# od-liu/CS3602-LLM-Inference-Acceleration

Hardware: NVIDIA B200
Metric: kv_compress_step_throughput (higher is better)
Workload: dtype bf16

## Files before the change

### cs3602-llm-inference-acceleration_b200/csrc/kvc_device.cuh

```cuda
#pragma once
#include <cuda_bf16.h>
#include <cuda_fp16.h>
#include <cuda_runtime.h>
#include <stdint.h>

#include <type_traits>

#include "kvc.h"

namespace kvc {

constexpr int kHistBits = 11;
constexpr int kHistBins = 1 << kHistBits;
constexpr int kMiscInts = 128;
constexpr int kMaxPoolHalo = 32;

constexpr int kMiscBin = 0;
constexpr int kMiscBelow = 1;
constexpr int kMiscMaxRaw = 2;
constexpr int kMiscWarpA = 32;
constexpr int kMiscWarpB = 64;
constexpr int kMiscHalo = 96;

struct CarryDev {
    char* acc;
    int64_t asb, ash;
    int32_t group, prev;
};
static_assert(sizeof(CarryDev) == 32, "CarryDev is part of the kernel parameters");

struct LayerDev {
    const char* k_in;
    const char* v_in;
    char* k_out;
    char* v_out;
    int32_t* idx_out;
    const int32_t* idx_in;
    int64_t ksb, ksh, kss;
    int64_t vsb, vsh, vss;
    int32_t S, sink, lo, hi, ksel, tail, score, pool;
    const char* n_in;
    int64_t nsb, nsh;
    CarryDev carry;
};
static_assert(sizeof(LayerDev) == 184, "LayerDev is passed by value in kernel params");

struct BatchDev {
    int32_t B, H;
    int32_t idx_cap;
    int32_t cpr;
    int32_t pad0, pad1;
    int32_t nsw;
    int32_t off_hist, off_idx, off_keys, off_stage;
    int32_t upc;
    char* ws;
    int64_t ws_unit;
    int64_t ws_keys;
    LayerDev layers[KVC_MAX_LAYERS_PER_LAUNCH];
};
static_assert(sizeof(BatchDev) < 32 * 1024, "kernel parameters are limited to 32 KB");

template <int DT>
struct Traits;
template <>
struct Traits<KVC_DTYPE_F32> {
    using Key = uint32_t;
    static constexpr int kElemBytes = 4;
    static constexpr int kKeyBits = 32;
    __device__ static __forceinline__ uint32_t to_raw(float x) { return __float_as_uint(x); }
    __device__ static __forceinline__ float from_raw(uint32_t r) { return __uint_as_float(r); }
    __device__ static __forceinline__ float sumsq(int4 v, float acc) {
        float a = __int_as_float(v.x), b = __int_as_float(v.y), c = __int_as_float(v.z), d = __int_as_float(v.w);
        acc = fmaf(a, a, acc);
        acc = fmaf(b, b, acc);
        acc = fmaf(c, c, acc);
        acc = fmaf(d, d, acc);
        return acc;
    }
};
template <>
struct Traits<KVC_DTYPE_BF16> {
    using Key = uint16_t;
    static constexpr int kElemBytes = 2;
    static constexpr int kKeyBits = 16;
    __device__ static __forceinline__ uint32_t to_raw(float x) {
        return (uint32_t)__bfloat16_as_ushort(__float2bfloat16_rn(x));
    }
    __device__ static __forceinline__ float from_raw(uint32_t r) { return __uint_as_float(r << 16); }
    __device__ static __forceinline__ float sumsq(int4 v, float acc) {
        const uint32_t w[4] = {(uint32_t)v.x, (uint32_t)v.y, (uint32_t)v.z, (uint32_t)v.w};
#pragma unroll
        for (int i = 0; i < 4; ++i) {
            float lo = __uint_as_float(w[i] << 16);
            float hi = __uint_as_float(w[i] & 0xffff0000u);
            acc = fmaf(lo, lo, acc);
            acc = fmaf(hi, hi, acc);
        }
        return acc;
    }
};
template <>
struct Traits<KVC_DTYPE_F16> {
    using Key = uint16_t;
    static constexpr int kElemBytes = 2;
    static constexpr int kKeyBits = 16;
    __device__ static __forceinline__ uint32_t to_raw(float x) {
        return (uint32_t)__half_as_ushort(__float2half_rn(x));
    }
    __device__ static __forceinline__ float from_raw(uint32_t r) {
        return __half2float(__ushort_as_half((unsigned short)r));
// ... 416 lines not shown
```

### cs3602-llm-inference-acceleration_b200/csrc/kvc_fused_tma.cuh

```cuda
#pragma once
#include "kvc_device.cuh"
#include "kvc_tma.cuh"

namespace kvc {

__host__ __device__ constexpr int swz_bits(int cpr) { return (cpr % 8 == 0) ? 3 : (cpr % 4 == 0) ? 2 : (cpr % 2 == 0) ? 1 : 0; }

template <int DT, int CPR>
__device__ __forceinline__ float row_sumsq_smem(uint32_t row_addr, int lane, int cpr) {
    using Tr = Traits<DT>;
    if constexpr (CPR == 0) {
        float tot = 0.f;
        for (int c = 0; c < cpr; ++c) {
            const float a = Tr::sumsq(lds128(row_addr + c * 16), 0.f);
            tot = (c == 0) ? a : tot + a;
        }
        return tot;
    } else {
        constexpr int SB = swz_bits(CPR);
        constexpr int G = 1 << SB;
        const int x = (lane >> (3 - SB)) & (G - 1);
        uint32_t base[G];
#pragma unroll
        for (int m = 0; m < G; ++m) base[m] = row_addr + (uint32_t)(((m ^ x) - m) * 16);
        float acc[CPR];
#pragma unroll
        for (int c = 0; c < CPR; ++c) acc[c] = Tr::sumsq(lds128(base[c & (G - 1)] + c * 16), 0.f);
        float tot = 0.f;
#pragma unroll
        for (int g = 0; g < CPR / G; ++g) {
#pragma unroll
            for (int s = 1; s < G; s <<= 1) {
#pragma unroll
                for (int m = 0; m < G; m += 2 * s) acc[g * G + m] += acc[g * G + m + s];
            }
            tot = (g == 0) ? acc[0] : tot + acc[g * G];
        }
        return tot;
    }
}

__device__ __forceinline__ void warp_load_rows(uint32_t slot, uint32_t bar, const char* src, int rows, bool dense,
                                               int lane, int rb) {
    const bool in = lane < rows;
    const unsigned long long a = (unsigned long long)src;
    const unsigned long long prev = __shfl_up_sync(0xffffffffu, a, 1);
    const bool head = in && (lane == 0 || !dense || a != prev + (unsigned)rb);
    const uint32_t heads = __ballot_sync(0xffffffffu, head);
    if (lane == 0) mbar_arrive_expect_tx(bar, (uint32_t)(rows * rb));
    __syncwarp();
    if (head) {
        const uint32_t later = heads & ~((2u << lane) - 1u);
        const int next = later ? (__ffs(later) - 1) : rows;
        bulk_g2s(slot + (uint32_t)(lane * rb), src, (uint32_t)((next - lane) * rb), bar);
    }
}

struct KeepMap {
    const int32_t* sidx;
    int sink, ksel, tail0;
    __device__ __forceinline__ int operator()(int j) const {
        return j < sink ? j : (j < sink + ksel ? sidx[j - sink] : j + tail0);
    }
};

template <typename Key, int NT>
__device__ __forceinline__ void carry_unit(const CarryDev& c, const KeepMap& src_row, int C, int b, int h) {
    char* base = c.acc + (int64_t)b * c.asb + (int64_t)h * c.group * c.ash;
    const int n = c.group * C;
    for (int e0 = 0; e0 < n; e0 += NT) {
        const int e = e0 + (int)threadIdx.x;
        Key* row = nullptr;
        int i = 0;
        Key val = 0;
        bool write = false;
        if (e < n) {
            const int g = e / C;
            i = e - g * C;
            const int s = src_row(i);
            row = reinterpret_cast<Key*>(base + (int64_t)g * c.ash);
            write = s != i || s >= c.prev;
            if (write && s < c.prev) val = row[s];
        }
        __syncthreads();
        if (write) row[i] = val;
    }
}

__device__ __forceinline__ void gather_unit(const KeepMap& src_row, int C, const char* kbase, const char* vbase,
                                            int64_t kss, int64_t vss, char* ko, char* vo, int rb, uint32_t slot,
                                            uint32_t bar, uint32_t& parity, int stage, int nstage, int lane) {
    const bool kdense = kss == rb, vdense = vss == rb;
    const int nbc = (C + 31) >> 5;
    for (int t = stage; t < 2 * nbc; t += nstage) {
        const bool isv = t >= nbc;
        const int j0 = (isv ? t - nbc : t) << 5;
        const int rows = min(32, C - j0);
        const int row = lane < rows ? src_row(j0 + lane) : 0;
        const char* src = isv ? vbase + (int64_t)row * vss : kbase + (int64_t)row * kss;
        warp_load_rows(slot, bar, src, rows, isv ? vdense : kdense, lane, rb);
        mbar_wait(bar, parity);
        parity ^= 1;
        if (lane == 0) {
            bulk_s2g((isv ? vo : ko) + (int64_t)j0 * rb, slot, (uint32_t)(rows * rb));
            bulk_commit();
            bulk_wait_read<0>();
        }
        __syncwarp();
    }
}

template <int DT, int NT>
__device__ __forceinline__ void keys_from_values(const typename Traits<DT>::Key* src, int R, int score,
                                                 typename Traits<DT>::Key* keys, uint32_t* hist, int32_t* misc) {
    using Tr = Traits<DT>;
    using Key = typename Tr::Key;
    constexpr int kShift0 = Tr::kKeyBits - kHistBits;
    const bool snap = (score == KVC_SCORE_SNAPKV_POOL);
    const bool desc = (score == KVC_SCORE_L2_HIGH);
    uint32_t local_max = 0;
    load_keys_vectorised<DT, NT>(src, R, keys, [&](int i, uint32_t raw) {
        if (snap) {
            keys[i] = (Key)raw;
            local_max = max(local_max, raw);
        } else {
            const Key key = ordered_key<Key>(raw, desc);
            keys[i] = key;
            atomicAdd(&hist[(uint32_t)key >> kShift0], 1u);
        }
    });
    if (snap) {
#pragma unroll
        for (int o = 16; o > 0; o >>= 1) local_max = max(local_max, __shfl_xor_sync(0xffffffffu, local_max, o));
        if ((threadIdx.x & 31) == 0) atomicMax(reinterpret_cast<uint32_t*>(&misc[kMiscMaxRaw]), local_max);
    }
}

template <int DT, int NT, typename Layer>
__device__ __forceinline__ void select_from_memory(const Layer& L, const typename Traits<DT>::Key* norm_row, int b, int bh,
                                                   typename Traits<DT>::Key* keys, uint32_t* hist, int32_t* misc,
                                                   int32_t* sidx) {
    using Key = typename Traits<DT>::Key;
    const int tid = threadIdx.x;
    const int R = L.hi - L.lo;
    if (L.score == KVC_SCORE_GIVEN_INDEX) {
        const int32_t* src = L.idx_in + (int64_t)bh * L.ksel;
        for (int i = tid; i < L.ksel; i += NT) sidx[i] = min(max(src[i], 0), L.S - 1);
        return;
    }
    for (int i = tid; i < kHistBins; i += NT) hist[i] = 0;
    if (tid == 0) misc[kMiscMaxRaw] = 0;
    __syncthreads();
    if (L.score == KVC_SCORE_GIVEN_SCORE || L.score == KVC_SCORE_GIVEN_SCORE_SHARED) {
        const Key* src = reinterpret_cast<const Key*>(L.idx_in) + (int64_t)(L.score == KVC_SCORE_GIVEN_SCORE ? bh : b) * R;
        load_keys_vectorised<DT, NT>(src, R, keys, [&](int i, uint32_t raw) { keys[i] = (Key)raw; });
        __syncthreads();
        snapkv_transform<DT, NT>(keys, R, L.pool, hist, misc, false);
    } else {
        keys_from_values<DT, NT>(norm_row + L.lo, R, L.score, keys, hist, misc);
        __syncthreads();
        if (L.score == KVC_SCORE_SNAPKV_POOL) snapkv_transform<DT, NT>(keys, R, L.pool, hist, misc);
    }
    block_radix_select<Key, NT>(keys, R, L.ksel, hist, misc, sidx, L.lo);
}

template <int DT, int CPR, int NT, int MINB>
__global__ void __launch_bounds__(NT, MINB) kvc_fused_tma_kernel(const __grid_constant__ BatchDev bd) {
    using Tr = Traits<DT>;
    using Key = typename Tr::Key;
    constexpr int kShift0 = Tr::kKeyBits - kHistBits;
    const int cpr = CPR > 0 ? CPR : bd.cpr;
    const int RB = cpr * 16;

    const int bx = blockIdx.x, by = blockIdx.y;
    const LayerDev& L = bd.layers[by];
    const int tid = threadIdx.x, lane = tid & 31, warp = tid >> 5;

    extern __shared__ __align__(128) unsigned char smem[];
    int32_t* misc = reinterpret_cast<int32_t*>(smem);
    uint32_t* hist = reinterpret_cast<uint32_t*>(smem + bd.off_hist);
    int32_t* sidx = reinterpret_cast<int32_t*>(smem + bd.off_idx);
    Key* keys = reinterpret_cast<Key*>(smem + bd.off_keys);
    const int nsw = bd.nsw;
    const bool stager = warp < nsw;
    const uint32_t slot = smem_u32(smem + bd.off_stage) + (uint32_t)(warp * 32 * RB);
    const uint32_t bar = smem_u32(smem + kMiscInts * 4) + (uint32_t)warp * 8;
    uint32_t parity = 0;

    const int R = L.hi - L.lo;
    const int ksel = L.ksel;
    const int score = L.score;
    const bool kdense = L.kss == RB;
    const bool given_score = score == KVC_SCORE_GIVEN_SCORE || score == KVC_SCORE_GIVEN_SCORE_SHARED;
    const bool by_value = given_score || L.n_in != nullptr;
    const bool scan = ksel > 0 && score != KVC_SCORE_GIVEN_INDEX && !by_value;

    if (stager) {
        if (lane == 0) {
            mbar_init(bar, 1);
            mbar_init_fence();
        }
        __syncwarp();
    }
    const int n_units = bd.B * bd.H;
    const int bh_end = min(n_units, (bx + 1) * bd.upc);
    for (int bh = bx * bd.upc; bh < bh_end; ++bh) {
    const int b = bh / bd.H, h = bh - b * bd.H;
    if (bd.ws != nullptr) {
        char* unit = bd.ws + ((int64_t)by * n_units + bh) * bd.ws_unit;
        keys = reinterpret_cast<Key*>(unit);
        sidx = reinterpret_cast<int32_t*>(unit + bd.ws_keys);
    }
    const char* kbase = L.k_in + (int64_t)b * L.ksb + (int64_t)h * L.ksh;
    const char* vbase = L.v_in + (int64_t)b * L.vsb + (int64_t)h * L.vsh;
    const char* kreg = kbase + (int64_t)L.lo * L.kss;
    const int nblk = (R + 31) >> 5;
    if (scan && stager && warp < nblk)
        warp_load_rows(slot, bar, kreg + (int64_t)(warp * 32 + lane) * L.kss, min(32, R - warp * 32), kdense, lane, RB);

    if (ksel > 0 && (score == KVC_SCORE_GIVEN_INDEX || by_value)) {
        const Key* norm_row = L.n_in ? reinterpret_cast<const Key*>(L.n_in + (int64_t)b * L.nsb + (int64_t)h * L.nsh)
                                     : nullptr;
        select_from_memory<DT, NT>(L, norm_row, b, bh, keys, hist, misc, sidx);
    } else if (ksel > 0) {
        for (int i = tid; i < kHistBins; i += NT) hist[i] = 0;
        if (tid == 0) misc[kMiscMaxRaw] = 0;
        __syncthreads();
        const bool snap = (score == KVC_SCORE_SNAPKV_POOL);
        const bool desc = (score == KVC_SCORE_L2_HIGH);
        uint32_t local_max = 0;
        if (stager) {
            for (int blk = warp; blk < nblk; blk += nsw) {
                const int r0 = blk << 5;
                const int rows = min(32, R - r0);
                mbar_wait(bar, parity);
                parity ^= 1;
                float ss = 0.f;
                if (lane < rows) ss = row_sumsq_smem<DT, CPR>(slot + (uint32_t)(lane * RB), lane, cpr);
                __syncwarp();
                const int nb = blk + nsw;
                if (nb < nblk)
                    warp_load_rows(slot, bar, kreg + (int64_t)(nb * 32 + lane) * L.kss, min(32, R - nb * 32), kdense,
                                   lane, RB);
                if (lane < rows) {
                    const uint32_t raw = Tr::to_raw(sqrtf(ss));
                    if (snap) {
                        keys[r0 + lane] = (Key)raw;
                        local_max = max(local_max, raw);
                    } else {
                        const Key key = ordered_key<Key>(raw, desc);
                        keys[r0 + lane] = key;
                        atomicAdd(&hist[(uint32_t)key >> kShift0], 1u);
                    }
                }
            }
        }
        if (snap) {
#pragma unroll
            for (int o = 16; o > 0; o >>= 1) local_max = max(local_max, __shfl_xor_sync(0xffffffffu, local_max, o));
            if (lane == 0) atomicMax(reinterpret_cast<uint32_t*>(&misc[kMiscMaxRaw]), local_max);
        }
        __syncthreads();
        if (snap) snapkv_transform<DT, NT>(keys, R, L.pool, hist, misc);
        block_radix_select<Key, NT>(keys, R, ksel, hist, misc, sidx, L.lo);
    }
    __syncthreads();

    const int C = L.sink + ksel + L.tail;
    const KeepMap src_row{sidx, L.sink, ksel, L.S - L.tail - L.sink - ksel};
    if (L.idx_out != nullptr) {
        int32_t* io = L.idx_out + (int64_t)bh * C;
        for (int j = tid; j < C; j += NT) io[j] = src_row(j);
    }
    if (L.carry.acc != nullptr) carry_unit<Key, NT>(L.carry, src_row, C, b, h);
    if (stager)
        gather_unit(src_row, C, kbase, vbase, L.kss, L.vss, L.k_out + (int64_t)bh * C * RB,
                    L.v_out + (int64_t)bh * C * RB, RB, slot, bar, parity, warp, nsw, lane);
    __syncthreads();
    }
}

}
```

### cs3602-llm-inference-acceleration_b200/csrc/kvc_sm100a.cu

```cuda
#include <algorithm>
#include <atomic>
#include <cstdio>
#include <cmath>
#include <cstdlib>
#include <cstring>
#include <mutex>
#include <type_traits>
#include <utility>
#include <vector>

#include <nvtx3/nvToolsExt.h>

#include "kvc_device.cuh"
#include "kvc_fused_tma.cuh"
#include "kvc_h2o.cuh"
#include "kvc_h2o_tc.cuh"
#include "kvc_slab.cuh"
#include "kvc_vote.cuh"

#ifndef KVC_PART
#define KVC_PART 127
#endif
#define KVC_HAS_CORE (KVC_PART & 1)
#define KVC_HAS_SLAB (KVC_PART & 2)
// ... 276 lines not shown
    int64_t keys = 0, unit = 0;
};
static WsLayout ws_layout(int dtype, int max_region, int idx_cap) {
    WsLayout w;
    w.keys = ((int64_t)max_region * key_bytes(dtype) + 15) & ~(int64_t)15;
    w.unit = w.keys + (((int64_t)idx_cap * 4 + 15) & ~(int64_t)15);
    return w;
}
static bool onchip_plan_ok(const TmaPlan& tp, int cpr, bool light_traffic) {
    if (!tp.ok) return false;
    if (light_traffic) return tp.slide_slots >= 2;
    return (long)tp.ctas * tp.nsw * 32 * cpr * 16 >= 48 * 1024;
}

#if KVC_HAS_CORE || KVC_HAS_FUSED_OTHER
template <int DT>
static FusedFn pick_tma_nt(int cpr, int nt) {
    return by_cpr(cpr, [&](auto c) {
        return nt == 512 ? FusedFn(kvc_fused_tma_kernel<DT, c, 512, 1>) : FusedFn(kvc_fused_tma_kernel<DT, c, 256, 3>);
    });
}
#endif
FusedFn pick_tma_bf16(int cpr, int nt);
FusedFn pick_tma_other(int dtype, int cpr, int nt);
#if KVC_HAS_CORE
FusedFn pick_tma_bf16(int cpr, int nt) { return pick_tma_nt<KVC_DTYPE_BF16>(cpr, nt); }
static FusedFn pick_tma(int dtype, int cpr, int nt) {
    return dtype == KVC_DTYPE_BF16 ? pick_tma_bf16(cpr, nt) : pick_tma_other(dtype, cpr, nt);
}
#endif
#if KVC_HAS_FUSED_OTHER
FusedFn pick_tma_other(int dtype, int cpr, int nt) {
    return dtype == KVC_DTYPE_F32 ? pick_tma_nt<KVC_DTYPE_F32>(cpr, nt) : pick_tma_nt<KVC_DTYPE_F16>(cpr, nt);
}
#endif

static int ensure_tma_attrs(const void* fn, int device) {
    static std::mutex mu;
    static std::vector<std::pair<const void*, int>> done;
    {
        std::lock_guard<std::mutex> lock(mu);
        for (const auto& d : done)
            if (d.first == fn && d.second == device) return KVC_OK;
    }
    cudaError_t e = cudaFuncSetAttribute(fn, cudaFuncAttributeMaxDynamicSharedMemorySize, (int)kMaxSmemOptin);
    if (e != cudaSuccess) return cuda_fail(e, "cudaFuncSetAttribute(max dynamic smem)");
    e = cudaFuncSetAttribute(fn, cudaFuncAttributePreferredSharedMemoryCarveout, (int)cudaSharedmemCarveoutMaxShared);
    if (e != cudaSuccess) return cuda_fail(e, "cudaFuncSetAttribute(carveout)");
    std::lock_guard<std::mutex> lock(mu);
    done.emplace_back(fn, device);
    return KVC_OK;
}


using SlabFn = void (*)(const SlabBatchDev);
using AppendFn = void (*)(const AppendBatchDev);
using AppendOneFn = void (*)(const AppendOneDev);
SlabFn pick_slab_bf16(int cpr, int nt);
SlabFn pick_slab_other(int dtype, int cpr, int nt);
AppendFn pick_append(int dtype, int cpr);
AppendOneFn pick_append_one(int dtype, int cpr);
AppendFn pick_append_tma(int dtype, int cpr);

#if KVC_HAS_SLAB || KVC_HAS_SLAB_OTHER
template <int DT>
static SlabFn pick_slab_nt(int cpr, int nt) {
    return by_cpr(cpr, [&](auto c) {
        return nt == 512 ? SlabFn(kvc_slab_compress_kernel<DT, c, 512, 1>) : SlabFn(kvc_slab_compress_kernel<DT, c, 256, 3>);
    });
}
#endif
#if KVC_HAS_SLAB
SlabFn pick_slab_bf16(int cpr, int nt) { return pick_slab_nt<KVC_DTYPE_BF16>(cpr, nt); }
static SlabFn pick_slab(int dtype, int cpr, int nt) {
    return dtype == KVC_DTYPE_BF16 ? pick_slab_bf16(cpr, nt) : pick_slab_other(dtype, cpr, nt);
}
#endif
#if KVC_HAS_SLAB_OTHER
SlabFn pick_slab_other(int dtype, int cpr, int nt) {
    return dtype == KVC_DTYPE_F32 ? pick_slab_nt<KVC_DTYPE_F32>(cpr, nt) : pick_slab_nt<KVC_DTYPE_F16>(cpr, nt);
}
#endif

#if KVC_HAS_APPEND
AppendOneFn pick_append_one(int dtype, int cpr) {
    return by_dtype(dtype, [&](auto dt) {
        return by_cpr(cpr, [&](auto c) { return AppendOneFn(kvc_slab_append_kernel<dt, c, AppendOneDev>); });
    });
}
AppendFn pick_append(int dtype, int cpr) {
    return by_dtype(dtype, [&](auto dt) {
        return by_cpr(cpr, [&](auto c) { return AppendFn(kvc_slab_append_kernel<dt, c, AppendBatchDev>); });
    });
}
AppendFn pick_append_tma(int dtype, int cpr) {
    return by_dtype(dtype, [&](auto dt) {
        return by_cpr(cpr, [&](auto c) { return AppendFn(kvc_slab_append_tma_kernel<dt, c>); });
    });
}
#endif

static int check_shape(const kvc_shape* shape, int* cpr_out) {
    if (!shape) return KVC_ERR_INVALID_ARG;
    const int B = shape->batch, H = shape->heads, D = shape->head_dim, dt = shape->dtype;
    if (B <= 0 || H <= 0 || D <= 0) return KVC_ERR_INVALID_ARG;
    if (dt != KVC_DTYPE_F32 && dt != KVC_DTYPE_F16 && dt != KVC_DTYPE_BF16) return KVC_ERR_UNSUPPORTED;
// ... 69 lines not shown
    WsLayout w;
};
static LaunchPlan plan_launch(int dtype, int cpr, const ChunkStats& s, bool light_traffic, bool in_place, int64_t units,
                              int64_t unit_bytes, bool may_use_ws) {
    LaunchPlan lp;
    lp.tp = plan_tma(dtype, cpr, s.max_region, s.idx_cap, s.any_select, light_traffic, units, unit_bytes, in_place);
    lp.ws = s.any_select && may_use_ws && !onchip_plan_ok(lp.tp, cpr, light_traffic);
    if (lp.ws) {
        lp.w = ws_layout(dtype, s.max_region, s.idx_cap);
        lp.tp = plan_tma(dtype, cpr, 0, 0, true, light_traffic);
    }
    return lp;
}

template <class Batch>
static int fill_batch(Batch& bd, const kvc_shape* shape, int cpr, const ChunkStats& s, const LaunchPlan& lp,
                      void* workspace, int64_t workspace_bytes) {
    if (lp.ws && lp.w.unit * shape->batch * shape->heads * s.n_active > workspace_bytes) return KVC_ERR_INVALID_ARG;
    if (!lp.tp.ok) return KVC_ERR_TOO_LARGE;
    memset(&bd, 0, sizeof(bd));
    bd.B = shape->batch;
    bd.H = shape->heads;
    bd.cpr = cpr;
    bd.idx_cap = s.idx_cap;
    if (lp.ws) {
        bd.ws = (char*)workspace;
        bd.ws_unit = lp.w.unit;
        bd.ws_keys = lp.w.keys;
    }
    bd.nsw = lp.tp.nsw;
    bd.off_hist = lp.tp.off_hist;
    bd.off_idx = lp.tp.off_idx;
    bd.off_keys = lp.tp.off_keys;
    bd.off_stage = lp.tp.off_stage;
    return KVC_OK;
}

template <class Layer>
static void fill_layer_plan(Layer& d, const kvc_layer_plan& p, const kvc_carry_layer* carry, int e) {
    d.S = p.seq_len;
    d.sink = p.sink;
    d.lo = p.sel_lo;
    d.hi = p.sel_hi;
    d.ksel = p.k_sel;
    d.tail = p.tail;
    d.score = p.k_sel > 0 ? p.score : KVC_SCORE_NONE;
    d.pool = p.pool_kernel;
    if (!carry || !carry->acc) return;
    d.carry.acc = (char*)carry->acc;
    d.carry.asb = carry->acc_stride_b * e;
    d.carry.ash = carry->acc_stride_h * e;
    d.carry.group = carry->group;
    d.carry.prev = carry->prev_len < p.seq_len ? carry->prev_len : p.seq_len;
}

}

using namespace kvc;

extern "C" {

#if KVC_HAS_CORE
int kvc_abi_version(void) { return KVC_ABI_VERSION; }

const char* kvc_build_info(void) {
    return "libkvc_sm100a: sm_100a, nvcc " KVC_STR(__CUDACC_VER_MAJOR__) "." KVC_STR(__CUDACC_VER_MINOR__);
}

const char* kvc_status_string(int status) {
    switch (status) {
        case KVC_OK: return "ok";
        case KVC_ERR_INVALID_ARG: return "invalid argument";
        case KVC_ERR_UNSUPPORTED: return "unsupported dtype / head_dim / alignment";
        case KVC_ERR_TOO_LARGE: return "selection region too large for the on-chip score buffer";
        case KVC_ERR_CUDA: return "CUDA error";
        default: return "unknown status";
    }
}

const char* kvc_last_cuda_error(void) { return g_last_error; }

int64_t kvc_launch_count(void) { return g_launches.load(); }

int32_t kvc_max_region_rows(int32_t dtype, int32_t k_sel) {
    if (dtype < 0 || dtype > 2 || k_sel < 0) return 0;
    const int64_t idx = ((int64_t)k_sel + 3) & ~(int64_t)3;
    const int64_t left = (int64_t)kMaxSmemOptin - kSmemFixed - idx * 4;
    if (left <= 0) return 0;
    const int64_t rows = (left & ~(int64_t)15) / key_bytes(dtype);
    return (int32_t)(rows > 0x7fffffff ? 0x7fffffff : rows);
}

int kvc_compress_layers(const kvc_shape* shape, int32_t n_layers, const kvc_layer_plan* plans,
                        const kvc_layer_io* io, void* stream) {
    return kvc_compress_layers_ws(shape, n_layers, plans, io, nullptr, 0, stream);
}

int64_t kvc_workspace_bytes(const kvc_shape* shape, int32_t n_layers, const kvc_layer_plan* plans) {
    int cpr = 0;
    if (check_shape(shape, &cpr) != KVC_OK || n_layers <= 0 || !plans || !row_width_ok(cpr)) return 0;
    const int64_t bh = (int64_t)shape->batch * shape->heads;
    int64_t need = 0;
    for_each_chunk(n_layers, [&](int l0, int nl) -> int {
        const ChunkStats s = chunk_stats(plans + l0, nullptr, nl);
        if (!s.any_select) return KVC_OK;
        const LaunchPlan lp = plan_launch(shape->dtype, cpr, s, false, false, bh * s.n_active,
// ... 47 lines not shown
        const int64_t C = (int64_t)p.sink + p.k_sel + p.tail;
        if (C == 0) continue;
        if (!x.k_in || !x.v_in || !x.k_out || !x.v_out) return KVC_ERR_INVALID_ARG;
        if (C * cpr * 2 > 0x7fffffffLL) return KVC_ERR_TOO_LARGE;
        const uintptr_t a = (uintptr_t)x.k_in | (uintptr_t)x.v_in | (uintptr_t)x.k_out | (uintptr_t)x.v_out;
        if (a & 15) return KVC_ERR_UNSUPPORTED;
        const int64_t s = (x.k_stride_b | x.k_stride_h | x.k_stride_s | x.v_stride_b | x.v_stride_h | x.v_stride_s);
        if ((s * e) & 15) return KVC_ERR_UNSUPPORTED;
    }
    DeviceGuard guard(shape->device);
    NvtxRange nvtx_range("kvc_compress_layers_ws");
    if (guard.status != KVC_OK) return guard.status;

    return for_each_chunk(n_layers, [&](int l0, int nl) -> int {
        const ChunkStats s = chunk_stats(plans + l0, io + l0, nl);
        if (s.n_active == 0) return KVC_OK;
        const bool light = s.any_select && !s.any_scan;
        const LaunchPlan lp = plan_launch(dt, cpr, s, light, false, (int64_t)B * H * s.n_active,
                                          s.rows_moved / s.n_active * cpr * 16, workspace != nullptr);
        BatchDev bd;
        int st = fill_batch(bd, shape, cpr, s, lp, workspace, workspace_bytes);
        if (st != KVC_OK) return st;
        bd.upc = lp.tp.upc;
        int m = 0;
        for (int l = l0; l < l0 + nl; ++l) {
            const kvc_layer_plan& p = plans[l];
            const kvc_layer_io& x = io[l];
            if (p.sink + p.k_sel + p.tail == 0) continue;
            LayerDev& d = bd.layers[m++];
            d.k_in = (const char*)x.k_in;
            d.v_in = (const char*)x.v_in;
            d.k_out = (char*)x.k_out;
            d.v_out = (char*)x.v_out;
            d.idx_out = x.idx_out;
            d.idx_in = (p.score == KVC_SCORE_GIVEN_SCORE || p.score == KVC_SCORE_GIVEN_SCORE_SHARED) ? (const int32_t*)x.score_in
                                                                                              : x.idx_in;
            d.ksb = x.k_stride_b * e;
            d.ksh = x.k_stride_h * e;
            d.kss = x.k_stride_s * e;
            d.vsb = x.v_stride_b * e;
            d.vsh = x.v_stride_h * e;
            d.vss = x.v_stride_s * e;
            if (ranked(p) && x.norms_in) {
                d.n_in = (const char*)x.norms_in;
                d.nsb = x.n_stride_b * key_bytes(dt);
                d.nsh = x.n_stride_h * key_bytes(dt);
            }
            fill_layer_plan(d, p, carry ? carry + l : nullptr, e);
        }
        FusedFn fn = pick_tma(dt, cpr, lp.tp.nt);
        dim3 grid((unsigned)(((int64_t)B * H + lp.tp.upc - 1) / lp.tp.upc), (unsigned)s.n_active, 1);
        st = ensure_tma_attrs((const void*)fn, shape->device);
        if (st != KVC_OK) return st;
        fn<<<grid, lp.tp.nt, lp.tp.smem, (cudaStream_t)stream>>>(bd);
        return launched("kvc_fused_tma_kernel launch");
    });
}

int kvc_key_norms(const kvc_shape* shape, const void* k_in, int64_t stride_b, int64_t stride_h, int64_t stride_s,
                  int32_t row_lo, int32_t row_hi, void* norms_out, void* stream) {
    if (!shape || !k_in || !norms_out || row_lo < 0 || row_hi < row_lo) return KVC_ERR_INVALID_ARG;
    const int B = shape->batch, H = shape->heads, D = shape->head_dim, dt = shape->dtype;
    if (B <= 0 || H <= 0 || D <= 0) return KVC_ERR_INVALID_ARG;
    if (dt != KVC_DTYPE_F32 && dt != KVC_DTYPE_F16 && dt != KVC_DTYPE_BF16) return KVC_ERR_UNSUPPORTED;
    const int e = elem_bytes(dt);
    if (((int64_t)D * e) % 16 != 0 || ((uintptr_t)k_in & 15)) return KVC_ERR_UNSUPPORTED;
    if (((stride_b | stride_h | stride_s) * e) & 15) return KVC_ERR_UNSUPPORTED;
    const int R = row_hi - row_lo;
    const int64_t total = (int64_t)B * H * R;
    if (total == 0) return KVC_OK;
    DeviceGuard guard(shape->device);
    NvtxRange nvtx_range("kvc_key_norms");
    if (guard.status != KVC_OK) return guard.status;
    const int cpr = D * e / 16;
    const int lpr = pow2_lanes(cpr), cpl = cpr / lpr;
    const int rpw = 32 / lpr;
    const int64_t warps_needed = (total + rpw - 1) / rpw;
    int64_t blocks = (warps_needed + 7) / 8;
    const int64_t cap = 148LL * 8 * 4;
    if (blocks > cap) blocks = cap;
    cudaStream_t s = (cudaStream_t)stream;
    const int64_t sb = stride_b * e, sh = stride_h * e, ss = stride_s * e;
    by_dtype(dt, [&](auto d) {
        kvc_norm_kernel<d><<<(unsigned)blocks, 256, 0, s>>>((const char*)k_in, sb, sh, ss, H, row_lo, R, total, lpr, cpl,
                                                            (typename Traits<d>::Key*)norms_out);
    });
    return launched("kvc_norm_kernel launch");
}

int kvc_select(int32_t dtype, int32_t device, const void* scores, int64_t n_rows, int32_t n, int32_t k,
               int32_t largest, int32_t* idx_out, void* stream) {
    if (!scores || !idx_out || n_rows < 0 || n < 0 || k < 0 || k > n) return KVC_ERR_INVALID_ARG;
    if (dtype != KVC_DTYPE_F32 && dtype != KVC_DTYPE_F16 && dtype != KVC_DTYPE_BF16) return KVC_ERR_UNSUPPORTED;
    if (n_rows == 0 || k == 0) return KVC_OK;
    if (n_rows > 0x7fffffffLL) return KVC_ERR_INVALID_ARG;
    const size_t smem = fused_smem_bytes(dtype, n, (k + 3) & ~3);
    if (smem > (size_t)kMaxSmemOptin) return KVC_ERR_TOO_LARGE;
    DeviceGuard guard(device);
    NvtxRange nvtx_range("kvc_select");
    if (guard.status != KVC_OK) return guard.status;
    return by_dtype(dtype, [&](auto d) -> int {
        const int st = ensure_smem((const void*)kvc_select_kernel<d, kNT>, smem);
        if (st != KVC_OK) return st;
        kvc_select_kernel<d, kNT><<<(unsigned)n_rows, kNT, smem, (cudaStream_t)stream>>>(
            (const typename Traits<d>::Key*)scores, n, k, largest, idx_out);
        return launched("kvc_select_kernel launch");
    });
// ... 655 lines not shown
```

### cs3602-llm-inference-acceleration_b200/csrc/kvc_tcgen05.cuh

```cuda
#pragma once
#include <cuda.h>
#include <cuda_runtime.h>
#include <stdint.h>

namespace kvc {

__device__ __forceinline__ void tmem_alloc(uint32_t smem_dst, uint32_t ncols) {
    asm volatile("tcgen05.alloc.cta_group::1.sync.aligned.shared::cta.b32 [%0], %1;" ::"r"(smem_dst), "r"(ncols) : "memory");
    asm volatile("tcgen05.relinquish_alloc_permit.cta_group::1.sync.aligned;" ::: "memory");
}
__device__ __forceinline__ void tmem_dealloc(uint32_t taddr, uint32_t ncols) {
    asm volatile("tcgen05.dealloc.cta_group::1.sync.aligned.b32 %0, %1;" ::"r"(taddr), "r"(ncols) : "memory");
}
__device__ __forceinline__ void tc_fence_before() { asm volatile("tcgen05.fence::before_thread_sync;" ::: "memory"); }
__device__ __forceinline__ void tc_fence_after() { asm volatile("tcgen05.fence::after_thread_sync;" ::: "memory"); }
__device__ __forceinline__ void umma_f16(uint32_t d_tmem, uint64_t a_desc, uint64_t b_desc, uint32_t idesc, uint32_t accumulate) {
    asm volatile(
        "{\n\t.reg .pred p;\n\t"
        "setp.ne.b32 p, %4, 0;\n\t"
        "tcgen05.mma.cta_group::1.kind::f16 [%0], %1, %2, %3, p;\n\t}"
        ::"r"(d_tmem), "l"(a_desc), "l"(b_desc), "r"(idesc), "r"(accumulate)
        : "memory");
}
__device__ __forceinline__ void umma_commit(uint32_t bar) {
    asm volatile("tcgen05.commit.cta_group::1.mbarrier::arrive::one.shared::cluster.b64 [%0];" ::"r"(bar) : "memory");
}
__device__ __forceinline__ void tmem_ld32(uint32_t taddr, uint32_t (&r)[32]) {
    asm volatile(
        "tcgen05.ld.sync.aligned.32x32b.x32.b32 "
        "{%0,%1,%2,%3,%4,%5,%6,%7,%8,%9,%10,%11,%12,%13,%14,%15,%16,%17,%18,%19,%20,%21,%22,%23,%24,%25,%26,%27,%28,%29,%30,%31}, [%32];"
        : "=r"(r[0]), "=r"(r[1]), "=r"(r[2]), "=r"(r[3]), "=r"(r[4]), "=r"(r[5]), "=r"(r[6]), "=r"(r[7]), "=r"(r[8]),
          "=r"(r[9]), "=r"(r[10]), "=r"(r[11]), "=r"(r[12]), "=r"(r[13]), "=r"(r[14]), "=r"(r[15]), "=r"(r[16]),
          "=r"(r[17]), "=r"(r[18]), "=r"(r[19]), "=r"(r[20]), "=r"(r[21]), "=r"(r[22]), "=r"(r[23]), "=r"(r[24]),
          "=r"(r[25]), "=r"(r[26]), "=r"(r[27]), "=r"(r[28]), "=r"(r[29]), "=r"(r[30]), "=r"(r[31])
        : "r"(taddr)
        : "memory");
    asm volatile("tcgen05.wait::ld.sync.aligned;" ::: "memory");
}

__device__ __forceinline__ void tmem_ld16_async(uint32_t taddr, uint32_t (&r)[16]) {
    asm volatile(
        "tcgen05.ld.sync.aligned.32x32b.x16.b32 {%0,%1,%2,%3,%4,%5,%6,%7,%8,%9,%10,%11,%12,%13,%14,%15}, [%16];"
        : "=r"(r[0]), "=r"(r[1]), "=r"(r[2]), "=r"(r[3]), "=r"(r[4]), "=r"(r[5]), "=r"(r[6]), "=r"(r[7]), "=r"(r[8]),
          "=r"(r[9]), "=r"(r[10]), "=r"(r[11]), "=r"(r[12]), "=r"(r[13]), "=r"(r[14]), "=r"(r[15])
        : "r"(taddr)
        : "memory");
}
__device__ __forceinline__ void tmem_ld_wait() { asm volatile("tcgen05.wait::ld.sync.aligned;" ::: "memory"); }

__device__ __forceinline__ uint64_t umma_smem_desc(uint32_t smem_addr, uint32_t lbo_bytes, uint32_t sbo_bytes) {
    uint64_t d = 0;
    d |= (uint64_t)((smem_addr >> 4) & 0x3fff);
    d |= (uint64_t)((lbo_bytes >> 4) & 0x3fff) << 16;
    d |= (uint64_t)((sbo_bytes >> 4) & 0x3fff) << 32;
    d |= (uint64_t)1 << 46;
    return d;
}
__host__ __device__ constexpr uint32_t umma_idesc_f16(int fmt , int m, int n) {
    return (1u << 4) | ((uint32_t)fmt << 7) | ((uint32_t)fmt << 10) | ((uint32_t)(n >> 3) << 17) | ((uint32_t)(m >> 4) << 24);
}
__device__ __forceinline__ uint64_t umma_smem_desc_sw32(uint32_t smem_addr) {
    uint64_t d = 0;
    d |= (uint64_t)((smem_addr >> 4) & 0x3fff);
    d |= (uint64_t)1 << 16;
    d |= (uint64_t)(256 >> 4) << 32;
    d |= (uint64_t)1 << 46;
    d |= (uint64_t)6 << 61;
    return d;
}
__device__ __forceinline__ uint64_t umma_smem_desc_sw128(uint32_t smem_addr) {
    uint64_t d = 0;
    d |= (uint64_t)((smem_addr >> 4) & 0x3fff);
    d |= (uint64_t)1 << 16;
    d |= (uint64_t)(1024 >> 4) << 32;
    d |= (uint64_t)1 << 46;
    d |= (uint64_t)2 << 61;
    return d;
}

__device__ __forceinline__ float ex2(float x) {
    float y;
    asm("ex2.approx.ftz.f32 %0, %1;" : "=f"(y) : "f"(x));
    return y;
}

__device__ __forceinline__ void mbar_arrive(uint32_t bar) {
    asm volatile("mbarrier.arrive.shared::cta.b64 _, [%0];" ::"r"(bar) : "memory");
}

__device__ __forceinline__ void tma_load_4d(uint32_t dst_smem, const CUtensorMap* map, int c0, int c1, int c2, int c3,
                                            uint32_t bar) {
    asm volatile(
        "cp.async.bulk.tensor.4d.shared::cluster.global.tile.mbarrier::complete_tx::bytes [%0], [%1, {%2, %3, %4, %5}], [%6];"
        ::"r"(dst_smem), "l"(map), "r"(c0), "r"(c1), "r"(c2), "r"(c3), "r"(bar)
        : "memory");
}

using EncodeTiledFn = CUresult (*)(CUtensorMap*, CUtensorMapDataType, cuuint32_t, void*, const cuuint64_t*,
                                   const cuuint64_t*, const cuuint32_t*, const cuuint32_t*, CUtensorMapInterleave,
                                   CUtensorMapSwizzle, CUtensorMapL2promotion, CUtensorMapFloatOOBfill);
static inline EncodeTiledFn tensor_map_encoder() {
// ... 28 lines not shown
```

### cs3602-llm-inference-acceleration_b200/csrc/kvc_tma.cuh

```cuda
#pragma once
#include <cuda_runtime.h>
#include <stdint.h>

namespace kvc {

__device__ __forceinline__ uint32_t smem_u32(const void* p) { return (uint32_t)__cvta_generic_to_shared(p); }

__device__ __forceinline__ void mbar_init(uint32_t bar, uint32_t count) {
    asm volatile("mbarrier.init.shared::cta.b64 [%0], %1;" ::"r"(bar), "r"(count) : "memory");
}
__device__ __forceinline__ void mbar_init_fence() { asm volatile("fence.mbarrier_init.release.cluster;" ::: "memory"); }

__device__ __forceinline__ void mbar_arrive_expect_tx(uint32_t bar, uint32_t bytes) {
    asm volatile("mbarrier.arrive.expect_tx.shared::cta.b64 _, [%0], %1;" ::"r"(bar), "r"(bytes) : "memory");
}

__device__ __forceinline__ bool mbar_try_wait(uint32_t bar, uint32_t parity) {
    uint32_t ok;
    asm volatile(
        "{\n\t.reg .pred p;\n\t"
        "mbarrier.try_wait.parity.shared::cta.b64 p, [%1], %2;\n\t"
        "selp.u32 %0, 1, 0, p;\n\t}"
        : "=r"(ok)
        : "r"(bar), "r"(parity)
        : "memory");
    return ok != 0;
}
__device__ __forceinline__ void mbar_wait(uint32_t bar, uint32_t parity) {
    while (!mbar_try_wait(bar, parity)) {
    }
}

__device__ __forceinline__ void bulk_g2s(uint32_t dst_smem, const void* src_gmem, uint32_t bytes, uint32_t bar) {
    asm volatile("cp.async.bulk.shared::cluster.global.mbarrier::complete_tx::bytes [%0], [%1], %2, [%3];" ::"r"(dst_smem),
                 "l"(src_gmem), "r"(bytes), "r"(bar)
                 : "memory");
}
__device__ __forceinline__ void bulk_s2g(void* dst_gmem, uint32_t src_smem, uint32_t bytes) {
    asm volatile("cp.async.bulk.global.shared::cta.bulk_group [%0], [%1], %2;" ::"l"(dst_gmem), "r"(src_smem), "r"(bytes)
                 : "memory");
}
__device__ __forceinline__ void bulk_commit() { asm volatile("cp.async.bulk.commit_group;" ::: "memory"); }
template <int N>
__device__ __forceinline__ void bulk_wait_read() {
    asm volatile("cp.async.bulk.wait_group.read %0;" ::"n"(N) : "memory");
}
__device__ __forceinline__ void fence_proxy_async_smem() { asm volatile("fence.proxy.async.shared::cta;" ::: "memory"); }

__device__ __forceinline__ int4 lds128(uint32_t addr) {
    int4 r;
    asm volatile("ld.shared.v4.s32 {%0,%1,%2,%3}, [%4];" : "=r"(r.x), "=r"(r.y), "=r"(r.z), "=r"(r.w) : "r"(addr));
    return r;
}

}
```

Before: 6446.

## Cache likely-selected key rows in tensor memory to skip re-gathering them

During the scoring scan, the fused kernel estimates a selection threshold from a sample of key norms. It stashes the rows likely to be kept in per-warp tensor memory columns, allocated with tcgen05. After selection, the cached rows are written straight to the output and the gather phase skips reloading those key rows from global memory. This saves global reads but adds tensor memory allocation, extra barriers and ballots, fragmented bulk stores, and a host occupancy check that can disable the path.

```diff
diff --git a/cs3602-llm-inference-acceleration_b200/csrc/kvc_device.cuh b/cs3602-llm-inference-acceleration_b200/csrc/kvc_device.cuh
--- a/cs3602-llm-inference-acceleration_b200/csrc/kvc_device.cuh
+++ b/cs3602-llm-inference-acceleration_b200/csrc/kvc_device.cuh
@@ -18,6 +18,9 @@
 constexpr int kMiscBin = 0;
 constexpr int kMiscBelow = 1;
 constexpr int kMiscMaxRaw = 2;
+constexpr int kMiscStoreT = 3;
+constexpr int kMiscStoreA = 4;
+constexpr int kMiscStoreB = 5;
 constexpr int kMiscWarpA = 32;
 constexpr int kMiscWarpB = 64;
 constexpr int kMiscHalo = 96;
@@ -49,13 +52,17 @@
     int32_t B, H;
     int32_t idx_cap;
     int32_t cpr;
-    int32_t pad0, pad1;
+    int32_t store;
+    int32_t off_store;
     int32_t nsw;
     int32_t off_hist, off_idx, off_keys, off_stage;
     int32_t upc;
     char* ws;
     int64_t ws_unit;
     int64_t ws_keys;
+#ifdef KVC_LAB
+    unsigned long long* lab_store_count;
+#endif
     LayerDev layers[KVC_MAX_LAYERS_PER_LAUNCH];
 };
 static_assert(sizeof(BatchDev) < 32 * 1024, "kernel parameters are limited to 32 KB");
diff --git a/cs3602-llm-inference-acceleration_b200/csrc/kvc_fused_tma.cuh b/cs3602-llm-inference-acceleration_b200/csrc/kvc_fused_tma.cuh
--- a/cs3602-llm-inference-acceleration_b200/csrc/kvc_fused_tma.cuh
+++ b/cs3602-llm-inference-acceleration_b200/csrc/kvc_fused_tma.cuh
@@ -1,5 +1,6 @@
 #pragma once
 #include "kvc_device.cuh"
+#include "kvc_tcgen05.cuh"
 #include "kvc_tma.cuh"
 
 namespace kvc {
@@ -40,19 +41,35 @@
     }
 }
 
+template <bool SKIP = false>
 __device__ __forceinline__ void warp_load_rows(uint32_t slot, uint32_t bar, const char* src, int rows, bool dense,
-                                               int lane, int rb) {
-    const bool in = lane < rows;
+                                               int lane, int rb, bool skip = false) {
     const unsigned long long a = (unsigned long long)src;
     const unsigned long long prev = __shfl_up_sync(0xffffffffu, a, 1);
-    const bool head = in && (lane == 0 || !dense || a != prev + (unsigned)rb);
-    const uint32_t heads = __ballot_sync(0xffffffffu, head);
-    if (lane == 0) mbar_arrive_expect_tx(bar, (uint32_t)(rows * rb));
-    __syncwarp();
-    if (head) {
-        const uint32_t later = heads & ~((2u << lane) - 1u);
-        const int next = later ? (__ffs(later) - 1) : rows;
-        bulk_g2s(slot + (uint32_t)(lane * rb), src, (uint32_t)((next - lane) * rb), bar);
+    if constexpr (SKIP) {
+        const bool in = lane < rows && !skip;
+        const uint32_t ins = __ballot_sync(0xffffffffu, in);
+        const bool prev_in = lane > 0 && ((ins >> (lane - 1)) & 1u);
+        const bool head = in && (!prev_in || !dense || a != prev + (unsigned)rb);
+        const uint32_t brk = __ballot_sync(0xffffffffu, head || !in);
+        if (lane == 0) mbar_arrive_expect_tx(bar, (uint32_t)(__popc(ins) * rb));
+        __syncwarp();
+        if (head) {
+            const uint32_t later = brk & ~((2u << lane) - 1u);
+            const int next = later ? (__ffs(later) - 1) : 32;
+            bulk_g2s(slot + (uint32_t)(lane * rb), src, (uint32_t)((next - lane) * rb), bar);
+        }
+    } else {
+        const bool in = lane < rows;
+        const bool head = in && (lane == 0 || !dense || a != prev + (unsigned)rb);
+        const uint32_t heads = __ballot_sync(0xffffffffu, head);
+        if (lane == 0) mbar_arrive_expect_tx(bar, (uint32_t)(rows * rb));
+        __syncwarp();
+        if (head) {
+            const uint32_t later = heads & ~((2u << lane) - 1u);
+            const int next = later ? (__ffs(later) - 1) : rows;
+            bulk_g2s(slot + (uint32_t)(lane * rb), src, (uint32_t)((next - lane) * rb), bar);
+        }
     }
 }
 
@@ -87,26 +104,66 @@
     }
 }
 
+template <bool SKIP = false>
 __device__ __forceinline__ void gather_unit(const KeepMap& src_row, int C, const char* kbase, const char* vbase,
                                             int64_t kss, int64_t vss, char* ko, char* vo, int rb, uint32_t slot,
-                                            uint32_t bar, uint32_t& parity, int stage, int nstage, int lane) {
+                                            uint32_t bar, uint32_t& parity, int stage, int nstage, int lane,
+                                            const uint32_t* stored = nullptr, int lo = 0) {
     const bool kdense = kss == rb, vdense = vss == rb;
     const int nbc = (C + 31) >> 5;
+    if constexpr (!SKIP) {
+        for (int t = stage; t < 2 * nbc; t += nstage) {
+            const bool isv = t >= nbc;
+            const int j0 = (isv ? t - nbc : t) << 5;
+            const int rows = min(32, C - j0);
+            const int row = lane < rows ? src_row(j0 + lane) : 0;
+            const char* src = isv ? vbase + (int64_t)row * vss : kbase + (int64_t)row * kss;
+            warp_load_rows(slot, bar, src, rows, isv ? vdense : kdense, lane, rb);
+            mbar_wait(bar, parity);
+            parity ^= 1;
+            if (lane == 0) {
+                bulk_s2g((isv ? vo : ko) + (int64_t)j0 * rb, slot, (uint32_t)(rows * rb));
+                bulk_commit();
+                bulk_wait_read<0>();
+            }
+            __syncwarp();
+        }
+    } else {
     for (int t = stage; t < 2 * nbc; t += nstage) {
         const bool isv = t >= nbc;
         const int j0 = (isv ? t - nbc : t) << 5;
         const int rows = min(32, C - j0);
-        const int row = lane < rows ? src_row(j0 + lane) : 0;
+        const int j = j0 + lane;
+        const int row = lane < rows ? src_row(j) : 0;
+        bool skip = false;
+        if (!isv && lane < rows && j >= src_row.sink && j < src_row.sink + src_row.ksel) {
+            const int rr = row - lo;
+            skip = (stored[rr >> 5] >> (rr & 31)) & 1u;
+        }
+        const uint32_t gone = __ballot_sync(0xffffffffu, skip);
         const char* src = isv ? vbase + (int64_t)row * vss : kbase + (int64_t)row * kss;
-        warp_load_rows(slot, bar, src, rows, isv ? vdense : kdense, lane, rb);
+        warp_load_rows<true>(slot, bar, src, rows, isv ? vdense : kdense, lane, rb, skip);
         mbar_wait(bar, parity);
         parity ^= 1;
-        if (lane == 0) {
-            bulk_s2g((isv ? vo : ko) + (int64_t)j0 * rb, slot, (uint32_t)(rows * rb));
-            bulk_commit();
-            bulk_wait_read<0>();
+        if (gone == 0) {
+            if (lane == 0) {
+                bulk_s2g((isv ? vo : ko) + (int64_t)j0 * rb, slot, (uint32_t)(rows * rb));
+                bulk_commit();
+                bulk_wait_read<0>();
+            }
+        } else {
+            const bool in = lane < rows && !skip;
+            const bool head = in && (lane == 0 || ((gone >> (lane - 1)) & 1u));
+            if (head) {
+                const uint32_t later = (gone | (rows < 32 ? ~0u << rows : 0u)) & ~((2u << lane) - 1u);
+                const int next = later ? (__ffs(later) - 1) : 32;
+                bulk_s2g(ko + (int64_t)j * rb, slot + (uint32_t)(lane * rb), (uint32_t)((next - lane) * rb));
+                bulk_commit();
+                bulk_wait_read<0>();
+            }
         }
         __syncwarp();
+    }
     }
 }
 
@@ -164,6 +221,107 @@
     block_radix_select<Key, NT>(keys, R, L.ksel, hist, misc, sidx, L.lo);
 }
 
+constexpr int kStoreCells = 64;
+constexpr int kStoreCpr = 10;
+constexpr int kStoreCols = 160;
+constexpr int kStoreSample = 256;
+
+__host__ __device__ constexpr bool key_store_layer(int score, int R, int ksel) {
+    return (score == KVC_SCORE_L2_LOW || score == KVC_SCORE_L2_HIGH) && R >= kStoreSample && 16 * ksel >= R;
+}
+__host__ __device__ constexpr int key_store_smem(int max_region) { return 8 * kStoreCells * 4 + (max_region + 31) / 32 * 4; }
+
+__device__ __forceinline__ uint32_t store_col(uint32_t ta, uint32_t tb, int warp, int c) {
+    const uint32_t lanes = (uint32_t)((warp & 3) * 32) << 16;
+    return lanes + (warp < 4 ? ta + c : (c < 48 ? ta + 80 + c : tb + (c - 48)));
+}
+
+__device__ __forceinline__ int nth_set_bit(uint32_t m, int k) {
+    int p = 0;
+#pragma unroll
+    for (int b = 16; b > 0; b >>= 1)
+        if (__popc(m & ((1u << (p + b)) - 1u)) <= k) p += b;
+    return p;
+}
+
+__device__ __forceinline__ void store_threshold(const uint16_t* keys, uint32_t key, int q, int32_t* misc) {
+    const uint32_t kk = key | (key << 16);
+    const uint4* v = reinterpret_cast<const uint4*>(keys);
+    int lt = 0, le = 0;
+#pragma unroll 4
+    for (int i = 0; i < kStoreSample / 8; ++i) {
+        const uint4 w = v[i];
+        lt += __popc(__vcmpltu2(w.x, kk)) + __popc(__vcmpltu2(w.y, kk)) + __popc(__vcmpltu2(w.z, kk)) +
+              __popc(__vcmpltu2(w.w, kk));
+        le += __popc(__vcmpleu2(w.x, kk)) + __popc(__vcmpleu2(w.y, kk)) + __popc(__vcmpleu2(w.z, kk)) +
+              __popc(__vcmpleu2(w.w, kk));
+    }
+    lt >>= 4;
+    le >>= 4;
+    if (lt <= q && q < le) misc[kMiscStoreT] = (int32_t)key;
+}
+
+__device__ __forceinline__ void store_admit(uint32_t m, int& ncells, uint32_t& tail, int blk, uint32_t slot, int lane,
+                                            int warp, uint32_t ta, uint32_t tb, int32_t* cell_row, uint32_t* stored) {
+    constexpr int kW = kStoreCpr * 4;
+    const int room = kStoreCells - ncells;
+    if (__popc(m) > room) m = room > 0 ? m & ((1u << nth_set_bit(m, room)) - 1u) : 0u;
+    if (lane == 0) stored[blk] = m;
+    const int cnt = __popc(m);
+    if (cnt == 0) return;
+    if (lane < cnt) cell_row[ncells + lane] = blk * 32 + nth_set_bit(m, lane);
+    const int w0 = ncells * kW, w1 = w0 + cnt * kW;
+    for (int c = w0 >> 5; c <= (w1 - 1) >> 5; ++c) {
+        const int x = c * 32 + lane;
+        uint32_t val = tail;
+        if (x >= w0 && x < w1) {
+            const int k = (x - w0) / kW;
+            val = lds32(slot + (uint32_t)(nth_set_bit(m, k) * (kStoreCpr * 16) + ((x - w0) - k * kW) * 4));
+        }
+        tmem_st1(store_col(ta, tb, warp, c), val);
+        tail = val;
+    }
+    tmem_st_wait();
+    ncells += cnt;
+}
+
+__device__ __forceinline__ int store_drain(int ncells, int32_t* cell_row, const int32_t* sidx, int ksel, int lo,
+                                           char* ko_sel, int lane, int warp, uint32_t ta, uint32_t tb) {
+    constexpr int kW = kStoreCpr * 4;
+    int written = 0;
+    for (int c = lane; c < ncells; c += 32) {
+        const int row = lo + cell_row[c];
+        int a = 0, b = ksel;
+        while (a < b) {
+            const int mid = (a + b) >> 1;
+            if (sidx[mid] < row) a = mid + 1;
+            else b = mid;
+        }
+        const bool kept = a < ksel && sidx[a] == row;
+        cell_row[c] = kept ? a : -1;
+        written += kept;
+    }
+#pragma unroll
+    for (int o = 16; o > 0; o >>= 1) written += __shfl_xor_sync(0xffffffffu, written, o);
+    __syncwarp();
+    const int words = ncells * kW;
+    for (int c0 = 0; c0 * 32 < words; c0 += 8) {
+        uint32_t v[8];
+        tmem_ld8_async(store_col(ta, tb, warp, c0), v);
+        tmem_ld_wait();
+#pragma unroll
+        for (int j = 0; j < 8; ++j) {
+            const int x = (c0 + j) * 32 + lane;
+            if (x < words) {
+                const int cell = x / kW;
+                const int pos = cell_row[cell];
+                if (pos >= 0) *reinterpret_cast<uint32_t*>(ko_sel + (int64_t)pos * (kStoreCpr * 16) + (x - cell * kW) * 4) = v[j];
+            }
+        }
+    }
+    return written;
+}
+
 template <int DT, int CPR, int NT, int MINB>
 __global__ void __launch_bounds__(NT, MINB) kvc_fused_tma_kernel(const __grid_constant__ BatchDev bd) {
     using Tr = Traits<DT>;
@@ -194,6 +352,12 @@
     const bool given_score = score == KVC_SCORE_GIVEN_SCORE || score == KVC_SCORE_GIVEN_SCORE_SHARED;
     const bool by_value = given_score || L.n_in != nullptr;
     const bool scan = ksel > 0 && score != KVC_SCORE_GIVEN_INDEX && !by_value;
+    constexpr bool kStoreForm = CPR == kStoreCpr && NT == 32 * 8 && sizeof(Key) == 2;
+    const bool store = kStoreForm && bd.store != 0 && scan && nsw == NT / 32 && bd.ws == nullptr &&
+                       key_store_layer(score, R, ksel);
+    int32_t* cell_row = reinterpret_cast<int32_t*>(smem + bd.off_store) + warp * kStoreCells;
+    uint32_t* stored = reinterpret_cast<uint32_t*>(smem + bd.off_store + 8 * kStoreCells * 4);
+    uint32_t ta = 0, tb = 0;
 
     if (stager) {
         if (lane == 0) {
@@ -217,6 +381,14 @@
     const int nblk = (R + 31) >> 5;
     if (scan && stager && warp < nblk)
         warp_load_rows(slot, bar, kreg + (int64_t)(warp * 32 + lane) * L.kss, min(32, R - warp * 32), kdense, lane, RB);
+    if (store && warp == 0 && bh == bx * bd.upc) {
+        tmem_alloc_keep_permit(smem_u32(&misc[kMiscStoreA]), 128);
+        tmem_alloc_keep_permit(smem_u32(&misc[kMiscStoreB]), kStoreCols - 128);
+        tmem_relinquish();
+        tc_fence_before();
+    }
+    int ncells = 0;
+    uint32_t tail = 0;
 
     if (ksel > 0 && (score == KVC_SCORE_GIVEN_INDEX || by_value)) {
         const Key* norm_row = L.n_in ? reinterpret_cast<const Key*>(L.n_in + (int64_t)b * L.nsb + (int64_t)h * L.nsh)
@@ -226,6 +398,11 @@
         for (int i = tid; i < kHistBins; i += NT) hist[i] = 0;
         if (tid == 0) misc[kMiscMaxRaw] = 0;
         __syncthreads();
+        if (store) {
+            tc_fence_after();
+            ta = (uint32_t)misc[kMiscStoreA];
+            tb = (uint32_t)misc[kMiscStoreB];
+        }
         const bool snap = (score == KVC_SCORE_SNAPKV_POOL);
         const bool desc = (score == KVC_SCORE_L2_HIGH);
         uint32_t local_max = 0;
@@ -237,6 +414,22 @@
                 parity ^= 1;
                 float ss = 0.f;
                 if (lane < rows) ss = row_sumsq_smem<DT, CPR>(slot + (uint32_t)(lane * RB), lane, cpr);
+                if constexpr (kStoreForm) {
+                    if (store) {
+                        const uint32_t key = lane < rows ? (uint32_t)ordered_key<Key>(Tr::to_raw(sqrtf(ss)), desc) : 0u;
+                        if (blk == warp) {
+                            keys[r0 + lane] = (Key)key;
+                            __syncthreads();
+                            store_threshold(reinterpret_cast<const uint16_t*>(keys), key,
+                                            min(kStoreSample - 1, (int)((int64_t)ksel * kStoreSample * 6 / (5 * R))),
+                                            misc);
+                            __syncthreads();
+                        }
+                        const uint32_t T = (uint32_t)misc[kMiscStoreT];
+                        store_admit(__ballot_sync(0xffffffffu, lane < rows && key <= T), ncells, tail, blk, slot, lane,
+                                    warp, ta, tb, cell_row, stored);
+                    }
+                }
                 __syncwarp();
                 const int nb = blk + nsw;
                 if (nb < nblk)
@@ -268,16 +461,46 @@
 
     const int C = L.sink + ksel + L.tail;
     const KeepMap src_row{sidx, L.sink, ksel, L.S - L.tail - L.sink - ksel};
+    if constexpr (kStoreForm) {
+        if (store) {
+            const int n = store_drain(ncells, cell_row, sidx, ksel, L.lo, L.k_out + ((int64_t)bh * C + L.sink) * RB, lane,
+                                      warp, ta, tb);
+#ifdef KVC_LAB
+            if (bd.lab_store_count != nullptr && lane == 0) {
+                atomicAdd(&bd.lab_store_count[0], (unsigned long long)n);
+                if (warp == 0) atomicAdd(&bd.lab_store_count[1], (unsigned long long)ksel);
+            }
+#else
+            (void)n;
+#endif
+        }
+    }
     if (L.idx_out != nullptr) {
         int32_t* io = L.idx_out + (int64_t)bh * C;
         for (int j = tid; j < C; j += NT) io[j] = src_row(j);
     }
     if (L.carry.acc != nullptr) carry_unit<Key, NT>(L.carry, src_row, C, b, h);
-    if (stager)
-        gather_unit(src_row, C, kbase, vbase, L.kss, L.vss, L.k_out + (int64_t)bh * C * RB,
-                    L.v_out + (int64_t)bh * C * RB, RB, slot, bar, parity, warp, nsw, lane);
+    if (stager) {
+        if (kStoreForm && store)
+            gather_unit<true>(src_row, C, kbase, vbase, L.kss, L.vss, L.k_out + (int64_t)bh * C * RB,
+                              L.v_out + (int64_t)bh * C * RB, RB, slot, bar, parity, warp, nsw, lane, stored, L.lo);
+        else
+            gather_unit(src_row, C, kbase, vbase, L.kss, L.vss, L.k_out + (int64_t)bh * C * RB,
+                        L.v_out + (int64_t)bh * C * RB, RB, slot, bar, parity, warp, nsw, lane);
+    }
     __syncthreads();
     }
-}
-
-}
+    if constexpr (kStoreForm) {
+        if (store) {
+            tc_fence_before();
+            __syncthreads();
+            tc_fence_after();
+            if (warp == 0) {
+                tmem_dealloc((uint32_t)misc[kMiscStoreA], 128);
+                tmem_dealloc((uint32_t)misc[kMiscStoreB], kStoreCols - 128);
+            }
+        }
+    }
+}
+
+}
diff --git a/cs3602-llm-inference-acceleration_b200/csrc/kvc_sm100a.cu b/cs3602-llm-inference-acceleration_b200/csrc/kvc_sm100a.cu
--- a/cs3602-llm-inference-acceleration_b200/csrc/kvc_sm100a.cu
+++ b/cs3602-llm-inference-acceleration_b200/csrc/kvc_sm100a.cu
@@ -352,6 +352,29 @@
     return KVC_OK;
 }
 
+static int resident_ctas(const void* fn, int device, int nt, size_t smem) {
+    struct Entry {
+        const void* fn;
+        int device, nt;
+        size_t smem;
+        int n;
+    };
+    static std::mutex mu;
+    static std::vector<Entry> done;
+    {
+        std::lock_guard<std::mutex> lock(mu);
+        for (const auto& d : done)
+            if (d.fn == fn && d.device == device && d.nt == nt && d.smem == smem) return d.n;
+    }
+    int n = 0;
+    if (cudaOccupancyMaxActiveBlocksPerMultiprocessor(&n, fn, nt, smem) != cudaSuccess) {
+        cudaGetLastError();
+        n = 0;
+    }
+    std::lock_guard<std::mutex> lock(mu);
+    done.push_back({fn, device, nt, smem, n});
+    return n;
+}
 
 using SlabFn = void (*)(const SlabBatchDev);
 using AppendFn = void (*)(const AppendBatchDev);
@@ -527,6 +550,27 @@
     d.carry.ash = carry->acc_stride_h * e;
     d.carry.group = carry->group;
     d.carry.prev = carry->prev_len < p.seq_len ? carry->prev_len : p.seq_len;
+}
+
+static bool plan_key_store(int dtype, int cpr, const LaunchPlan& lp, const kvc_layer_plan* plans, const kvc_layer_io* io,
+                           int nl, int max_region, const void* fn, int device, size_t* smem, int* off_store) {
+    if (dtype == KVC_DTYPE_F32 || cpr != kStoreCpr || lp.ws || lp.tp.nt != 256 || lp.tp.nsw != 8) return false;
+    if (env_int("KVC_KEY_STORE", 1) == 0) return false;
+    bool any = false;
+    for (int l = 0; l < nl && !any; ++l)
+        any = ranked(plans[l]) && !io[l].norms_in &&
+              key_store_layer(plans[l].score, plans[l].sel_hi - plans[l].sel_lo, plans[l].k_sel);
+    if (!any) return false;
+    const int off = (int)((lp.tp.smem + 15) & ~(size_t)15);
+    const size_t need = (size_t)off + (size_t)key_store_smem(max_region);
+    int limit = kSmemPerSM / lp.tp.ctas - 1024;
+    if (limit > kMaxSmemOptin) limit = kMaxSmemOptin;
+    if (need > (size_t)limit) return false;
+    const int resident = resident_ctas(fn, device, lp.tp.nt, need);
+    if (resident < 1 || resident * kStoreCols > 512) return false;
+    *smem = need;
+    *off_store = off;
+    return true;
 }
 
 }
@@ -680,7 +724,16 @@
         dim3 grid((unsigned)(((int64_t)B * H + lp.tp.upc - 1) / lp.tp.upc), (unsigned)s.n_active, 1);
         st = ensure_tma_attrs((const void*)fn, shape->device);
         if (st != KVC_OK) return st;
-        fn<<<grid, lp.tp.nt, lp.tp.smem, (cudaStream_t)stream>>>(bd);
+        size_t smem = lp.tp.smem;
+        bd.store = plan_key_store(dt, cpr, lp, plans + l0, io + l0, nl, s.max_region, (const void*)fn, shape->device,
+                                  &smem, &bd.off_store) ? 1 : 0;
+#ifdef KVC_LAB
+        {
+            const char* c = getenv("KVC_STORE_COUNT");
+            bd.lab_store_count = (c && *c) ? (unsigned long long*)strtoull(c, nullptr, 16) : nullptr;
+        }
+#endif
+        fn<<<grid, lp.tp.nt, smem, (cudaStream_t)stream>>>(bd);
         return launched("kvc_fused_tma_kernel launch");
     });
 }
diff --git a/cs3602-llm-inference-acceleration_b200/csrc/kvc_tcgen05.cuh b/cs3602-llm-inference-acceleration_b200/csrc/kvc_tcgen05.cuh
--- a/cs3602-llm-inference-acceleration_b200/csrc/kvc_tcgen05.cuh
+++ b/cs3602-llm-inference-acceleration_b200/csrc/kvc_tcgen05.cuh
@@ -7,6 +7,12 @@
 
 __device__ __forceinline__ void tmem_alloc(uint32_t smem_dst, uint32_t ncols) {
     asm volatile("tcgen05.alloc.cta_group::1.sync.aligned.shared::cta.b32 [%0], %1;" ::"r"(smem_dst), "r"(ncols) : "memory");
+    asm volatile("tcgen05.relinquish_alloc_permit.cta_group::1.sync.aligned;" ::: "memory");
+}
+__device__ __forceinline__ void tmem_alloc_keep_permit(uint32_t smem_dst, uint32_t ncols) {
+    asm volatile("tcgen05.alloc.cta_group::1.sync.aligned.shared::cta.b32 [%0], %1;" ::"r"(smem_dst), "r"(ncols) : "memory");
+}
+__device__ __forceinline__ void tmem_relinquish() {
     asm volatile("tcgen05.relinquish_alloc_permit.cta_group::1.sync.aligned;" ::: "memory");
 }
 __device__ __forceinline__ void tmem_dealloc(uint32_t taddr, uint32_t ncols) {
@@ -47,6 +53,17 @@
         : "memory");
 }
 __device__ __forceinline__ void tmem_ld_wait() { asm volatile("tcgen05.wait::ld.sync.aligned;" ::: "memory"); }
+
+__device__ __forceinline__ void tmem_ld8_async(uint32_t taddr, uint32_t (&r)[8]) {
+    asm volatile("tcgen05.ld.sync.aligned.32x32b.x8.b32 {%0,%1,%2,%3,%4,%5,%6,%7}, [%8];"
+                 : "=r"(r[0]), "=r"(r[1]), "=r"(r[2]), "=r"(r[3]), "=r"(r[4]), "=r"(r[5]), "=r"(r[6]), "=r"(r[7])
+                 : "r"(taddr)
+                 : "memory");
+}
+__device__ __forceinline__ void tmem_st1(uint32_t taddr, uint32_t r) {
+    asm volatile("tcgen05.st.sync.aligned.32x32b.x1.b32 [%0], {%1};" ::"r"(taddr), "r"(r) : "memory");
+}
+__device__ __forceinline__ void tmem_st_wait() { asm volatile("tcgen05.wait::st.sync.aligned;" ::: "memory"); }
 
 __device__ __forceinline__ uint64_t umma_smem_desc(uint32_t smem_addr, uint32_t lbo_bytes, uint32_t sbo_bytes) {
     uint64_t d = 0;
diff --git a/cs3602-llm-inference-acceleration_b200/csrc/kvc_tma.cuh b/cs3602-llm-inference-acceleration_b200/csrc/kvc_tma.cuh
--- a/cs3602-llm-inference-acceleration_b200/csrc/kvc_tma.cuh
+++ b/cs3602-llm-inference-acceleration_b200/csrc/kvc_tma.cuh
@@ -47,6 +47,11 @@
 }
 __device__ __forceinline__ void fence_proxy_async_smem() { asm volatile("fence.proxy.async.shared::cta;" ::: "memory"); }
 
+__device__ __forceinline__ uint32_t lds32(uint32_t addr) {
+    uint32_t r;
+    asm volatile("ld.shared.b32 %0, [%1];" : "=r"(r) : "r"(addr));
+    return r;
+}
 __device__ __forceinline__ int4 lds128(uint32_t addr) {
     int4 r;
     asm volatile("ld.shared.v4.s32 {%0,%1,%2,%3}, [%4];" : "=r"(r.x), "=r"(r.y), "=r"(r.z), "=r"(r.w) : "r"(addr));
```

Result: slower. 5610, median of 6 (-13.0%).
